# Nielsencu/primal-ppo

Hardware: AMD Instinct MI355X
Metric: agent-steps/sec (env.step+observe) at 4096 envs×8 agents, 1/2/4/8 GPU (higher is better)
Workload: dtype int32; 1 GPU; c2: 4096 envs x 8 agents per GPU, 20x20 warehouse, FOV 11, 6 channels, random policy, env.step+observe; num_envs_per_gpu=4096, num_agents=8, fov=11, channels=6, human=Human (random goals, device A*), goals=lifelong, random, keep_bfs=True, total_envs=4096, parallelism=env-shards x1

## Files before the change

primal-ppo_amd/csrc/mapf_fused_rollout.inc:

```
    extern __shared__ __attribute__((aligned(16))) char smem[];
    constexpr int E = 4;
    constexpr bool TAPE = rollout_pol(POL) == ROLLOUT_TAPE, DESCENT = rollout_pol(POL) == ROLLOUT_DESCENT, PIBT = rollout_pol(POL) == ROLLOUT_PIBT;
    constexpr bool NOISE = rollout_pol_noise(POL);
    const int nb = (int)gridDim.x;
    const int wg = (ro.xcd_remap && (nb & 7) == 0) ? ((int)blockIdx.x & 7) * (nb >> 3) + ((int)blockIdx.x >> 3)
                                                   : (int)blockIdx.x;
    const int sub = SUBS > 1 ? __builtin_amdgcn_readfirstlane((int)(threadIdx.x >> 8)) : 0;
    const int qt = (int)(threadIdx.x & 255);
    const int blk = wg * SUBS + sub;
    const int b0 = blk * E;
    const int nenv = min(E, e.B - b0);
    const int le = qt >> 6;
    char *qsm = smem + (SUBS > 1 ? (size_t)sub * ro.sub_lds : 0);
    uint32_t *prog = reinterpret_cast<uint32_t *>(smem + (size_t)SUBS * ro.sub_lds);
    static_assert(SUBS == 1 || 4 * SUBS == PACE_RING, "the pacing ring takes the place of the per-wave counters");
    const int gw = sub * E + le;
    ObsLds L{};
    if constexpr (PERF) {
        L.rowsz = e.Hp * e.WW;
        L.mapc = reinterpret_cast<uint32_t *>(qsm);
    } else {
        L = obs_layout(e, E, qsm, true);
    }
    const size_t obs_sz = PERF ? rollout_perf_map_lds(e) : rollout_obs_lds(e);
    const size_t base_sz = PERF ? rollout_perf_lds_bytes(e, ROLLOUT_RANDOM) : rollout_lds_bytes(e, ROLLOUT_RANDOM);
    float4 *lut = reinterpret_cast<float4 *>(qsm + rollout_obs_lds(e) - 256);
    if (!PERF && qt < 16) lut[qt] = make_float4((float)(qt & 1), (float)((qt >> 1) & 1), (float)((qt >> 2) & 1), (float)(qt >> 3));
    if (SUBS > 1 && (int)threadIdx.x < 4 * SUBS)
        prog[threadIdx.x] = ro.fair <= 0 || wg * SUBS * E + (int)threadIdx.x < e.B ? 0u : 0xFFFFFFFFu;
    __syncthreads();
    if constexpr (!PERF) L.lut = lut;
    const size_t swl = srch::wave_lds<uint32_t, 1>(e.H, e.W);
    char *slds = qsm + obs_sz + (size_t)le * swl;
    uint32_t *lpath = reinterpret_cast<uint32_t *>(qsm + obs_sz + 4 * swl) + (size_t)le * e.Lmax;
    int32_t *trow = nullptr;
    if constexpr (TAPE) trow = reinterpret_cast<int32_t *>(qsm + base_sz) + (size_t)le * TAPE_K * 8;
    if constexpr (DESCENT || PIBT) trow = reinterpret_cast<int32_t *>(qsm + base_sz) + (size_t)le * 8;
    const uint32_t mreg = obs_map_word(e, b0, nenv, (int)(threadIdx.x & 63));
    EnvRegs rs{};
    if (le < nenv) env_regs_load<8>(e, b0 + le, rs, lpath);
    uint32_t pseen = 0, psince = 0;
    if constexpr (PIBT) {
        if (le < nenv) {
            const size_t ag = (size_t)(b0 + le) * e.N + (size_t)min((int)(threadIdx.x & 63) >> 3, e.N - 1);
            pseen = static_cast<const RO &>(ro).pibt_seen[ag];
            psince = static_cast<const RO &>(ro).pibt_since[ag];
        }
    }
    [[maybe_unused]] PerfAcc pacc;
    if constexpr (PERF) {
        if (le < nenv) pacc = perf_acc_load(ro_perf(ro) + (b0 + __builtin_amdgcn_readfirstlane(le)), ro_accumulate(ro));
    }
    if constexpr (PERF) __builtin_amdgcn_s_waitcnt(0xC07F);
    __builtin_amdgcn_s_waitcnt(0x0F70);
    uint32_t band_mask = 0;
    bool band_moves = false;
    if constexpr (BAND == OBS_BAND) {
        band_moves = ((size_t)e.B * e.N * e.C * e.F * e.F * 4) % MAPF_BAND_UNIT != 0;
        if (le < nenv && !band_moves)
            band_mask = obs_band_skip_mask(e, MAPF_BAND_UNIT, (size_t)(ro.obs + (size_t)(b0 + le) * e.N * e.C * e.F * e.F),
                                           (int)(threadIdx.x & 63));
    }
    if constexpr (PERF) {
        if (le < nenv && (int)(threadIdx.x & 63) < L.rowsz) L.mapc[(size_t)le * L.rowsz + (threadIdx.x & 63)] = mreg;
        __builtin_amdgcn_fence(__ATOMIC_ACQ_REL, "wavefront");
        __builtin_amdgcn_wave_barrier();
    }
    RSTAMP_BEGIN();
    const bool pacing = SUBS > 1 && ro.slack >= 0 && __builtin_amdgcn_readfirstlane(le) < nenv;
    const bool fair = SUBS > 1 && ro.fair > 0 && le < nenv;
    const int live = min(max(e.B - wg * SUBS * E, 0), 4 * SUBS);
    for (int t = 0; t < T; ++t) {
        const DevEnv &E = e;
        const RO &R = ro;
        if (pacing) {
            RSTAMP_WAIT0();
            pace_wait(prog, t, R.slack, live);
            RSTAMP_WAIT1();
        }
        if (fair) {
            if ((uint32_t)t > group_min(prog, 4 * SUBS) + (uint32_t)R.fair) __builtin_amdgcn_s_setprio(0);
            else __builtin_amdgcn_s_setprio(2);
        }
        const size_t BN = (size_t)E.B * E.N;
        const size_t s = R.slots ? (size_t)t : 0;
        [[maybe_unused]] uint32_t *sp_words = nullptr;
        if constexpr (BAND == OBS_SPARSE) {
            const int lew = __builtin_amdgcn_readfirstlane(le);
            sp_words = ro_shadow(ro) + (s * (size_t)E.B + (size_t)(b0 + lew)) * OBS_SPARSE_WORDS;
            band_mask = 0xFFFFFFFFu;
            if (t < ro_valid(ro) && lew < nenv) band_mask = obs_sparse_old(sp_words, (int)(threadIdx.x & 63));
        }
        if constexpr (TAPE) {
            if ((t & (TAPE_K - 1)) == 0) {
                if (le < nenv) {
                    int lane = (int)(threadIdx.x & 63);
                    asm volatile("" : "+v"(lane));
                    const int i = lane & 7, r0 = lane >> 3, nrow = min(TAPE_K, T - t);
                    const int32_t *src = R.actions + ((size_t)(t + r0) * E.B + (size_t)(b0 + le)) * E.N + i;
                    int32_t v[TAPE_K / 8];
#pragma unroll
                    for (int k = 0; k < TAPE_K / 8; ++k)
                        v[k] = (i < E.N && r0 + 8 * k < nrow) ? src[(size_t)(8 * k) * BN] : 0;
#pragma unroll
                    for (int k = 0; k < TAPE_K / 8; ++k) as_lds(trow)[lane + 64 * k] = v[k];
                }
                __builtin_amdgcn_fence(__ATOMIC_ACQ_REL, "wavefront");
                __builtin_amdgcn_wave_barrier();
            }
        }
        if constexpr (DESCENT) {
            __builtin_amdgcn_fence(__ATOMIC_ACQUIRE, "wavefront");
            if (le < nenv) {
                int lane = (int)(threadIdx.x & 63);
                asm volatile("" : "+v"(lane));
                const int i = lane >> 3;
                const bool head = (lane & 7) == 0 && i < E.N;
                int a = 0;
                if (head) {
                    const size_t ai = (size_t)(b0 + le) * E.N + i;
                    a = descent_action(E, E.bfs + ai * bfs_cells(E.H, E.W), rs.pi, rs.clock, i);
                    if (!PERF || R.actions) R.actions[s * BN + ai] = a;
                }
                if constexpr (NOISE)
                    a = noise_play_wave(E.seed, E.env_offset + (uint32_t)(b0 + le), rs.clock, E.noise_q16, E.N, head, i, a);
                if (head) as_lds(trow)[i] = a;
            }
            __builtin_amdgcn_fence(__ATOMIC_ACQ_REL, "wavefront");
            __builtin_amdgcn_wave_barrier();
        }
        if constexpr (PIBT) {
            __builtin_amdgcn_fence(__ATOMIC_ACQUIRE, "wavefront");
            if (le < nenv) {
                int lane = (int)(threadIdx.x & 63);
                asm volatile("" : "+v"(lane));
                const int i = lane >> 3;
                const bool head = (lane & 7) == 0 && i < E.N;
                const size_t ai = (size_t)(b0 + le) * E.N + (size_t)min(i, E.N - 1);
                uint32_t cand[NA] = {PIBT_NONE, PIBT_NONE, PIBT_NONE, PIBT_NONE, PIBT_NONE};
                uint32_t age = 0;
                if (head) {
                    age = pibt_age(pseen, psince, rs.gi, rs.clock);
                    const unsigned sm = E.smask[(E.shared_map ? 0 : (size_t)(b0 + le) * E.H * E.W) + prow(rs.pi) * E.W + pcol(rs.pi)];
                    pibt_candidates(E, E.bfs + ai * bfs_cells(E.H, E.W), rs.pi, sm, rs.hp, rs.hn, rs.clock, i, cand, [&](int j) {
                        return (uint32_t)__builtin_amdgcn_readfirstlane(
                            (int)human_ahead(as_lds(rs.lp), rs.hs, rs.hcur ? rs.hlen1 : rs.hlen0, j));
                    });
                }
                int a = pibt_solve_wave<8>(E.N, lane, head ? rs.pi : NO_CELL, cand, age);
                if (head && (!PERF || R.actions)) R.actions[s * BN + ai] = a;
                if constexpr (NOISE)
                    a = noise_play_wave(E.seed, E.env_offset + (uint32_t)(b0 + le), rs.clock, E.noise_q16, E.N, head, i, a);
                if (head) as_lds(trow)[i] = a;
            }
            __builtin_amdgcn_fence(__ATOMIC_ACQ_REL, "wavefront");
            __builtin_amdgcn_wave_barrier();
        }
        StepOut o = PERF ? StepOut{} : R.out;
        if (o.status) o.status += s * BN;
        if (o.reward) o.reward += s * BN;
        if (o.shadow_goals) o.shadow_goals += s * E.B;
        if (o.cost) o.cost += s * BN;
        if (o.train_valid) o.train_valid += s * BN * NA;
        if (o.actions_fixed) o.actions_fixed += s * BN;
        if (o.goals_reached) o.goals_reached += s * BN;
        if (o.constraints) o.constraints += s * BN;
        if (o.reward_total) o.reward_total += s * BN;
        PairsDeferred dfr;
        [[maybe_unused]] StepVals pv;
        step_pairs_env<8, !PERF, true, true, TAPE || DESCENT || PIBT, PERF>(
            E, TAPE ? trow + (size_t)(t & (TAPE_K - 1)) * 8 : (DESCENT || PIBT ? trow : (PERF && !R.actions ? nullptr : R.actions + s * BN)), o,
            TAPE || DESCENT || PIBT ? 1u : 3u, 0,
            blk * 256 + qt, L, b0, RegMap{mreg, true}, dfr, &rs, PERF ? &pv : nullptr);
        if constexpr (PERF) {
            if (le < nenv) {
                perf_acc_step<8>(pacc, pv, E.N, (int)(threadIdx.x & 63));
                step_pairs_search_inline(E, dfr, slds, L.mapc + (size_t)le * L.rowsz, rs);
            }
        } else
        if (le < nenv) {
            const ObsGroup g = obs_wave_init(E, L, le, mreg);
            if (BAND == OBS_BAND && band_moves)
                band_mask = obs_band_skip_mask(E, MAPF_BAND_UNIT,
                                               (size_t)(R.obs + (s * BN + (size_t)(b0 + le) * E.N) * E.C * E.F * E.F),
                                               (int)(threadIdx.x & 63));
            float *ob;
            if constexpr (ST == OBS_BITS) ob = R.obs + s * BN * (size_t)obs_bits_words(E.C, E.F);
            else ob = R.obs + s * BN * E.C * E.F * E.F;
            obs_emit<false, ST, BAND, PIBT ? 0 : OBS_NT_GROUP>(E, L, ob, R.vec + s * BN * 4, g, b0, false, band_mask);
            if constexpr (BAND == OBS_SPARSE) obs_sparse_store(g.stream, L.swe, sp_words, (int)(threadIdx.x & 63));
            step_pairs_search_inline(E, dfr, slds, L.mapc + (size_t)le * L.rowsz, rs);
            if (pacing) pace_arrive(prog, t);
            else if (fair) publish_count(prog + gw, (uint32_t)(t + 1));
        }
        __builtin_amdgcn_fence(__ATOMIC_ACQ_REL, "wavefront");
        __builtin_amdgcn_wave_barrier();
    }
    if (le < nenv) env_regs_store<8>(e, b0 + le, rs);
    if constexpr (PIBT) {
        const int lane = (int)(threadIdx.x & 63);
        if (le < nenv && (lane & 7) == 0 && (lane >> 3) < e.N) {
            static_cast<const RO &>(ro).pibt_seen[(size_t)(b0 + le) * e.N + (lane >> 3)] = pseen;
            static_cast<const RO &>(ro).pibt_since[(size_t)(b0 + le) * e.N + (lane >> 3)] = psince;
        }
    }
    if constexpr (PERF) {
        if (le < nenv) perf_acc_store(pacc, ro_perf(ro) + (b0 + le), (int)(threadIdx.x & 63));
    }
    if (le < nenv) RSTAMP_END(b0 + le);
```

primal-ppo_amd/csrc/mapf_observe.h:

```cpp
#pragma once
#include "mapf_common.h"
#include "mapf_obs_bits.h"

namespace mapf {

constexpr int OBS_PLAIN = 0, OBS_NT = 1, OBS_BITS = 2;

struct ObsLds {
    int swe;
    uint32_t *stream, *occ, *mapc, *spos, *sgoal, *shn, *shp;
    int32_t *shpn;
    uint8_t *idg;
    uint32_t *bfsw;
    int32_t *bfsown;
    const float4 *lut;
    int stream_words, rowsz;
    bool bfs_win;
};

__host__ __device__ inline int obs_stream_words(const DevEnv &e, int E) { return (E * e.N * e.C * e.F * e.F + 31) / 32 + 1; }

__host__ __device__ inline bool obs_bfs_windows(const DevEnv &e) { return e.C >= 7 && e.keep_bfs && (e.W & 1) == 0; }
__host__ __device__ inline int obs_bfs_wd(const DevEnv &e) { return (e.F + 2) >> 1; }

// ... 122 lines not shown
    if (u0 < o) return false;
    const uint32_t r0 = u0 - o, r1 = r0 + (uint32_t)unit;
    const uint32_t k = r0 / ab;
    return r0 >= k * ab + 4u * (uint32_t)z0 && r1 <= k * ab + 4u * (uint32_t)z1;
}
__host__ __device__ inline int obs_band_iters(const DevEnv &e) { return ((e.N * e.C * e.F * e.F) / 4 + 63) / 64; }
__host__ __device__ inline uint32_t obs_band_skip_mask(const DevEnv &e, int unit, size_t off, int lane) {
    const int nq = (e.N * e.C * e.F * e.F) >> 2;
    uint32_t m = 0;
    for (int k = 0, q = lane; q < nq && k < 32; ++k, q += 64)
        if (obs_band_skip(e, unit, off, q)) m |= 1u << k;
    return m;
}
#ifndef MAPF_BAND_UNIT
#define MAPF_BAND_UNIT 64
#endif

__device__ inline void obs_zero_band_store(const DevEnv &e, float *__restrict__ obs, size_t k0, size_t k1, size_t t,
                                           size_t nt) {
    int z0, z1;
    if (!obs_zero_band(e, z0, z1)) return;
    const size_t CFF = (size_t)e.C * e.F * e.F;
    float4 *o4 = reinterpret_cast<float4 *>(obs);
    const float4 zero = make_float4(0.f, 0.f, 0.f, 0.f);
    for (size_t idx = k0 * 32 + t; idx < k1 * 32; idx += nt) {
        const size_t k = idx >> 5, j = idx & 31;
        const size_t qa = (k * CFF + z0 + 3) >> 2, qb = (k * CFF + z1) >> 2;
        if (qa + j < qb) o4[qa + j] = zero;
    }
}

constexpr int OBS_BAND = 1, OBS_SPARSE = 2;
constexpr int OBS_SPARSE_WORDS = 16, OBS_SPARSE_PIECE = 16;
__host__ __device__ inline bool obs_sparse_applies(int N, int C, int F, size_t obs_addr) {
    const int fl = N * C * F * F;
    return fl > 0 && fl % OBS_SPARSE_PIECE == 0 && fl / OBS_SPARSE_PIECE <= 32 * OBS_SPARSE_WORDS && (obs_addr & 63) == 0;
}
__device__ inline uint32_t obs_sparse_old(const uint32_t *words, int lane) {
    typedef const __attribute__((address_space(4))) uint32_t cu32;
    cu32 *w = (cu32 *)(uintptr_t)words;
    const int g = lane >> 2;
    uint32_t a = 0;
#pragma unroll
    for (int j = 0; j < OBS_SPARSE_WORDS; ++j) a |= ((w[j] >> g) & 0x10001u) << j;
    return a;
}
__device__ inline void obs_sparse_store(const uint32_t *stream, int swe, uint32_t *words, int lane) {
    uint32_t b = 0;
#pragma unroll
    for (int i = 0; i < 4; ++i) {
        const int idx = 4 * lane + i;
        const uint32_t w = idx < swe ? stream[idx] : 0u;
        b |= (((w & 0xFFFFu) ? 1u : 0u) | ((w >> 16) ? 2u : 0u)) << (2 * i);
    }
    b |= (uint32_t)__shfl_down((int)b, 1) << 8;
    b |= (uint32_t)__shfl_down((int)b, 2) << 16;
    if ((lane & 3) == 0) words[lane >> 2] = b;
}

struct ObsGroup {
    int tid, nt;
    int le0, nenv;
    uint32_t *stream;
    const uint32_t *mapc;
    bool wave;
#ifdef MAPF_STAMPS
    int diag = 0;
#endif
};

__device__ inline void obs_sync(const ObsGroup &g) {
    if (g.wave) {
        __builtin_amdgcn_fence(__ATOMIC_ACQ_REL, "wavefront");
        __builtin_amdgcn_wave_barrier();
    } else {
        __syncthreads();
    }
}

__device__ inline ObsGroup obs_workgroup(const ObsLds &L, int nenv) {
    return ObsGroup{(int)threadIdx.x, (int)blockDim.x, 0, nenv, L.stream, L.mapc, false};
}

__device__ inline ObsGroup obs_wave_init(const DevEnv &e, const ObsLds &L, int le, uint32_t mreg) {
    const int lane = lane_id();
    uint32_t *st = L.stream + (size_t)le * L.swe;
    for (int k = lane; k < L.swe; k += 64) st[k] = 0u;
    for (int k = lane; k < L.rowsz; k += 64) L.occ[le * L.rowsz + k] = 0u;
    uint32_t *mp = L.mapc + le * L.rowsz;
    if (lane < L.rowsz) mp[lane] = mreg;
    ObsGroup g{lane, 64, le, 1, st, mp, true};
    obs_sync(g);
    return g;
}

constexpr int OBS_NT_GROUP = 4;
constexpr uint32_t OBS_NT_DROP = 0x80000000u;
constexpr int OBS_NT_AUX = 16 | 2;
#ifndef MAPF_STORE_PRED
#define MAPF_STORE_PRED 0
#endif

template <int BAND, bool WHOLE, int GN>
__device__ __forceinline__ void obs_nt_group(__amdgpu_buffer_rsrc_t rs, const float4 *lut, const uint32_t *swp, int sh,
                                             int hsh, uint32_t voff, uint32_t mask, int cnt) {
    typedef uint32_t v4u __attribute__((ext_vector_type(4)));
    uint32_t sw[GN], vo[GN];
    float4 f[GN];
#pragma unroll
    for (int j = 0; j < GN; ++j) sw[j] = (WHOLE || j < cnt) ? swp[8 * j] : 0u;
#pragma unroll
    for (int j = 0; j < GN; ++j) {
        bool skip = false;
        if constexpr (BAND == OBS_BAND) skip = (mask >> j) & 1u;
        if constexpr (BAND == OBS_SPARSE)
            skip = (__builtin_amdgcn_ubfe(sw[j], hsh, 16) | __builtin_amdgcn_ubfe(mask, (j & 1) * 16 + (j >> 1), 1)) == 0;
        vo[j] = skip ? OBS_NT_DROP : voff;
        if constexpr (BAND != 0) asm("" : "+v"(vo[j]));
    }
#pragma unroll
    for (int j = 0; j < GN; ++j)
        if (WHOLE || j < cnt) f[j] = lut[__builtin_amdgcn_ubfe(sw[j], sh, 4)];
#pragma unroll
    for (int j = 0; j < GN; ++j) {
        if (!(WHOLE || j < cnt)) continue;
        const v4u d = {__float_as_uint(f[j].x), __float_as_uint(f[j].y), __float_as_uint(f[j].z), __float_as_uint(f[j].w)};
#if MAPF_STORE_PRED
        if (vo[j] != OBS_NT_DROP) __builtin_amdgcn_raw_buffer_store_b128(d, rs, voff + 1024u * j, 0, OBS_NT_AUX);
#else
        __builtin_amdgcn_raw_buffer_store_b128(d, rs, vo[j] + 1024u * j, 0, OBS_NT_AUX);
#endif
    }
}

template <int BAND, int GN>
__device__ __forceinline__ void obs_store_wave_nt(const float4 *lut, const uint32_t *swp, int sh, int hsh, float *dst, int q,
                                                  int lane, uint32_t band_mask) {
    const uintptr_t a = reinterpret_cast<uintptr_t>(dst);
    const uint32_t lo = (uint32_t)__builtin_amdgcn_readfirstlane((int)(uint32_t)a);
    const uint32_t hi = (uint32_t)__builtin_amdgcn_readfirstlane((int)(uint32_t)(a >> 32));
    q = __builtin_amdgcn_readfirstlane(q);
    const __amdgpu_buffer_rsrc_t rs =
        __builtin_amdgcn_make_buffer_rsrc(reinterpret_cast<void *>(((uintptr_t)hi << 32) | lo), 0, q * 16, 0x00020000);
    const int iters = (q + 63) >> 6;
    uint32_t voff = (uint32_t)lane * 16u;
    static_assert(GN == OBS_NT_GROUP, "an even group (the sparse mask's layout) within the immediate offset");
    for (int g = 0; g < iters / GN; ++g) {
        obs_nt_group<BAND, true, GN>(rs, lut, swp, sh, hsh, voff, band_mask, GN);
        swp += 8 * GN;
        voff += 1024u * GN;
        band_mask >>= BAND == OBS_SPARSE ? GN / 2 : GN;
    }
    if (iters % GN) obs_nt_group<BAND, false, GN>(rs, lut, swp, sh, hsh, voff, band_mask, iters % GN);
}

template <bool BFSCH = true, int ST = OBS_PLAIN, int BAND = 0, int GN = 0>
__device__ inline void obs_emit(const DevEnv &e, const ObsLds &L, float *__restrict__ obs, float *__restrict__ vec,
                                const ObsGroup &G, int b0, bool skip_band = false, uint32_t band_mask = 0) {
    using namespace obsd;
    const int N = e.N, F = e.F, C = e.C, FF = F * F, CFF = C * FF;
    const int K = G.nenv * N;
    const int kw = G.le0 * N;
    const int rowsz = L.rowsz;
    const int tid = G.tid, nt = G.nt;
    uint32_t *stream = G.stream;
    b0 += G.le0;
    const int E = G.nenv;

    const int HW = e.H * e.W;
#ifdef MAPF_STAMPS
    const int KB = G.diag == 3 ? 0 : K;
#else
    const int KB = K;
#endif
    for (int k = tid; k < KB; k += nt) {
        const int le = G.le0 + k / N;
        const int r = prow(L.spos[kw + k]), c = pcol(L.spos[kw + k]);
        const int rr = r + e.P, cc = c + e.P;
        atomicOr(&L.occ[le * rowsz + rr * e.WW + (cc >> 5)], 1u << (cc & 31));
        L.idg[le * HW + r * e.W + c] = (uint8_t)(k % N);
    }
    const int half = F / 2;
    const size_t bcells = bfs_cells(e.H, e.W);
    if (BFSCH && L.bfs_win) {
        const int WD = obs_bfs_wd(e);
        for (int idx = tid; idx < KB * F * WD; idx += nt) {
            const int task = idx / WD, w = idx - task * WD;
            const int k = task / F, y = task - k * F;
            const int rr = min(max(prow(L.spos[kw + k]) - half + y, 0), e.H - 1);
            const int col = min(max(((pcol(L.spos[kw + k]) - half) & ~1) + 2 * w, 0), e.W - 2);
            const int16_t *bm = e.bfs + ((size_t)b0 * N + k) * bcells;
            L.bfsw[kw * F * WD + idx] = *reinterpret_cast<const uint32_t *>(bm + bfs_at(e.W, rr, col));
        }
        for (int k = tid; k < KB; k += nt)
            L.bfsown[kw + k] = e.bfs[((size_t)b0 * N + k) * bcells + bfs_at(e.W, prow(L.spos[kw + k]), pcol(L.spos[kw + k]))];
    }
    obs_sync(G);

    const int R2 = e.R * e.R;
    for (int task = tid; task < KB * F; task += nt) {
        const int k = task / F, y = task - k * F;
        const int le = G.le0 + k / N;
        const int pr = prow(L.spos[kw + k]), pc = pcol(L.spos[kw + k]);
        const int tr = pr - half, tc = pc - half;
        const int rr = tr + y;
        const int prow_idx = rr + e.P;
        const uint32_t *mrow = G.mapc + (e.shared_map ? 0 : (le - G.le0) * rowsz) + prow_idx * e.WW;
        const uint32_t *orow = L.occ + le * rowsz + prow_idx * e.WW;
        uint32_t seg0 = seg_at(mrow, e.WW, tc + e.P, F);
        uint32_t segA = seg_at(orow, e.WW, tc + e.P, F);
        const uint32_t self = (y == half) ? (1u << half) : 0u;
        const int base = k * CFF + y * F;
        or_bits(stream, base, seg0 | self, F);
        or_bits(stream, base + FF, segA & ~self, F);
        for (uint32_t others = segA & ~self; others; others &= others - 1u) {
            const int cc = tc + __builtin_ctz(others);
            const int kj = le * N + L.idg[le * HW + rr * e.W + cc];
            const int xr = min(max(prow(L.sgoal[kj]), tr), tr + F - 1);
            const int xc = min(max(pcol(L.sgoal[kj]), tc), tc + F - 1);
            set_bit(stream, k * CFF + 3 * FF + (xr - tr) * F + (xc - tc));
        }
        if (e.use_da && rr >= 0 && rr < e.H) {
            const uint32_t hn = L.shn[le];
            const int dy = prow(hn) - rr;
            if (dy * dy <= R2) {
                const int w = isqrt_floor(R2 - dy * dy);
                int c0 = max(max(pcol(hn) - w, 0), tc), c1 = min(min(pcol(hn) + w, e.W - 1), tc + F - 1);
                if (c0 <= c1) {
                    const uint32_t m = ((1u << (c1 - c0 + 1)) - 1u) << (c0 - tc);
                    or_bits(stream, base + 4 * FF, m, F);
                }
            }
        }
        if (BFSCH && L.bfs_win && rr >= 0 && rr < e.H) {
            const int own = L.bfsown[kw + k];
            const uint32_t *win = L.bfsw + ((size_t)kw * F + task) * obs_bfs_wd(e);
            const int c0 = tc & ~1;
            uint32_t m = 0;
            for (int x = 0; x < F; ++x) {
                const int cc = tc + x, wi = cc - c0;
                const int v = (int16_t)(win[wi >> 1] >> ((wi & 1) * 16));
                if (cc >= 0 && cc < e.W && v >= 0 && v < own) m |= 1u << x;
            }
            if (own < 0) m = 0;
            or_bits(stream, base + 6 * FF, m, F);
        } else if (BFSCH && C >= 7 && e.keep_bfs && rr >= 0 && rr < e.H) {
            const size_t ai = (size_t)b0 * N + k;
            const int16_t *bm = e.bfs + ai * bcells;
            const int own = bm[bfs_at(e.W, pr, pc)];
            const int c0 = tc & ~1, cmax = bfs_tw(e.W) * 8 - 2;
            uint32_t wv[9];
#pragma unroll
            for (int w = 0; w < 9; ++w)
                if (2 * w < F + 1)
                    wv[w] = *reinterpret_cast<const uint32_t *>(bm + bfs_at(e.W, rr, min(max(c0 + 2 * w, 0), cmax)));
            uint32_t m = 0;
#pragma unroll
            for (int x = 0; x < 16; ++x) {
                const int cc = tc + x, wi = cc - c0;
                if (x < F) {
                    const int v = (int16_t)(wv[wi >> 1] >> ((wi & 1) * 16));
                    if (cc >= 0 && cc < e.W && v >= 0 && v < own) m |= 1u << x;
                }
            }
            if (own < 0) m = 0;
            or_bits(stream, base + 6 * FF, m, F);
        }
    }

    for (int k = tid; k < KB; k += nt) {
        const int le = G.le0 + k / N;
        const int pr = prow(L.spos[kw + k]), pc = pcol(L.spos[kw + k]);
        const int tr = pr - half, tc = pc - half;
        const int base = k * CFF;
        const int gr = prow(L.sgoal[kw + k]), gc = pcol(L.sgoal[kw + k]);
        if (tr <= gr && gr < tr + F && tc <= gc && gc < tc + F) set_bit(stream, base + 2 * FF + (gr - tr) * F + (gc - tc));
        const uint32_t hn = L.shn[le];
        const int hr = prow(hn), hc = pcol(hn);
        if (tr <= hr && hr < tr + F && tc <= hc && hc < tc + F) set_bit(stream, base + 4 * FF + (hr - tr) * F + (hc - tc));
        for (int q = 0; q < L.shpn[le]; ++q) {
            const uint32_t cell = L.shp[le * e.k_predict + q];
            const int r = prow(cell), c = pcol(cell);
            if (tr <= r && r < tr + F && tc <= c && c < tc + F) set_bit(stream, base + 5 * FF + (r - tr) * F + (c - tc));
        }
        const int dx = gr - pr, dy = gc - pc;
        const int d2 = dx * dx + dy * dy;
        float4 v;
        if (d2 == 0) {
            v = make_float4(0.f, 0.f, 0.f, 0.f);
        } else {
            const double d = __builtin_sqrt((double)d2);
            v = make_float4((float)((double)dx / d), (float)((double)dy / d), (float)d, 0.f);
        }
        reinterpret_cast<float4 *>(vec)[(size_t)b0 * N + k] = v;
    }
    obs_sync(G);
    TL_STAMP(4);
#ifdef MAPF_STAMPS
    if (G.diag == 2) return;
#endif

    if constexpr (ST == OBS_BITS) {
        const int WPA = obs_bits_words(C, F), nw = K * WPA;
        uint32_t *dw = reinterpret_cast<uint32_t *>(obs) + (size_t)b0 * N * WPA;
        if (((N * WPA) & 3) == 0 && ((uintptr_t)dw & 15) == 0) {
            for (int q = tid; q < (nw >> 2); q += nt) {
                int k = (4 * q) / WPA, w = 4 * q - k * WPA;
                uint32_t v[4];
#pragma unroll
                for (int j = 0; j < 4; ++j) {
                    v[j] = obs_bits_word(stream, CFF, k, w);
                    if (++w == WPA) { w = 0; ++k; }
                }
                reinterpret_cast<uint4 *>(dw)[q] = make_uint4(v[0], v[1], v[2], v[3]);
            }
        } else {
            for (int i = tid; i < nw; i += nt) {
                const int k = i / WPA;
                dw[i] = obs_bits_word(stream, CFF, k, i - k * WPA);
            }
        }
        return;
    }
    const size_t total = (size_t)K * CFF;
    float *dst = obs + (size_t)b0 * N * CFF;
    if (G.wave && L.lut && !skip_band && ((K * CFF) & 3) == 0) {
        const int sh = (tid & 7) * 4;
        const uint32_t *swp = stream + (tid >> 3);
        if constexpr (ST == OBS_NT && GN != 0) {
            obs_store_wave_nt<BAND, GN>(L.lut, swp, sh, (tid & 4) * 4, dst, (K * CFF) >> 2, tid, band_mask);
            return;
        }
        float4 *dp = reinterpret_cast<float4 *>(dst) + tid;
        [[maybe_unused]] int it = 0;
#pragma unroll 4
        for (int rem = ((K * CFF) >> 2) - tid; rem > 0; rem -= 64) {
            const uint32_t sw = *swp;
            const float4 f = L.lut[__builtin_amdgcn_ubfe(sw, sh, 4)];
            bool skip = false;
            if constexpr (BAND == OBS_BAND) skip = band_mask & 1u;
            if constexpr (BAND == OBS_SPARSE)
                skip = (__builtin_amdgcn_ubfe(sw, (tid & 4) * 4, 16) | __builtin_amdgcn_ubfe(band_mask, (it & 1) * 16 + (it >> 1), 1)) == 0;
            if (skip) {
            } else if constexpr (ST == OBS_NT) {
                typedef float v4f __attribute__((ext_vector_type(4)));
#if defined(MAPF_SLOT_STORE) && MAPF_SLOT_STORE == 1
                __builtin_nontemporal_store(v4f{f.x, f.y, f.z, f.w}, reinterpret_cast<v4f *>(dp));
#elif defined(MAPF_SLOT_STORE) && MAPF_SLOT_STORE == 2
                asm volatile("global_store_dwordx4 %0, %1, off sc1\n\ts_nop 1" ::"v"(dp), "v"(v4f{f.x, f.y, f.z, f.w}) : "memory");
#elif defined(MAPF_SLOT_STORE) && MAPF_SLOT_STORE == 3
                *dp = f;
#else
// ... 65 lines not shown
```

primal-ppo_amd/csrc/mapf_step_pairs.h:

```cpp
#pragma once
#include "mapf_group.h"
#include "mapf_kernels.h"
#include "mapf_observe.h"
#include "mapf_pyset.h"

namespace mapf {

namespace pairs {

__device__ inline unsigned abit(int r, int c) {
    if (r == 0 && c == 0) return 1u;
    if (r == 0 && c == 1) return 1u << 1;
    if (r == 1 && c == 0) return 1u << 2;
    if (r == 0 && c == -1) return 1u << 3;
    if (r == -1 && c == 0) return 1u << 4;
    return 0u;
}
__device__ inline unsigned keys_of(int r, int c) {
    unsigned m = 0;
#pragma unroll
    for (int t = 0; t < NA; ++t)
        if (abs(dr(t) - r) + abs(dc(t) - c) <= 1) m |= 1u << t;
    return m;
}
// ... 19 lines not shown
struct EnvRegs {
    uint32_t pi, pj, gi;
    int la;
    float creg;
    uint32_t clock, hp, hn, hng, hgoal, hstart, hentr, replans;
    int hs, hcur, hlen0, hlen1;
    uint32_t *lp;
};

__device__ inline void env_regs_path_to_lds(const DevEnv &e, int b, int buf, int len, uint32_t *lp) {
    const uint32_t *p = human_path(e, b, buf);
    for (int k = lane_id(); k < len; k += 64) lp[k] = p[k];
    __builtin_amdgcn_fence(__ATOMIC_ACQ_REL, "wavefront");
    __builtin_amdgcn_wave_barrier();
}

template <int NP>
__device__ inline void env_regs_load(const DevEnv &e, int b, EnvRegs &r, uint32_t *lp) {
    const int lane = lane_id(), i = lane / NP, j = lane % NP;
    const bool vi = i < e.N, vj = j < e.N;
    const size_t ai = (size_t)b * e.N + i, aj = (size_t)b * e.N + j;
    r.pi = vi ? e.pos[ai] : 0u;
    r.pj = vj ? e.pos[aj] : 0u;
    r.gi = vi ? e.goal[ai] : 0u;
    r.la = vi ? (int)e.last_act[ai] : -1;
    const int RR = e.R * e.R;
    r.creg = RR < 64 ? e.cost_lut[lane <= RR ? lane : 0] : 0.f;
    r.clock = e.clock[b];
    r.hentr = e.hentr[b];
    r.hp = e.hpos[b];
    r.hn = e.hnext[b];
    r.hng = e.hnext_goal[b];
    r.hgoal = e.hgoal[b];
    r.hstart = e.hnext_start[b];
    r.replans = 0u;
    r.hs = e.hstep[b];
    r.hcur = e.hcur[b];
    r.hlen0 = e.hlen[(size_t)b * 2];
    r.hlen1 = e.hlen[(size_t)b * 2 + 1];
    r.lp = lp;
    env_regs_path_to_lds(e, b, r.hcur, r.hcur ? r.hlen1 : r.hlen0, lp);
}

template <int NP>
__device__ inline void env_regs_store(const DevEnv &e, int b, const EnvRegs &r) {
    const int lane = lane_id(), i = lane / NP, j = lane % NP;
    if (i < e.N && j == 0) {
        const size_t ai = (size_t)b * e.N + i;
        e.pos[ai] = r.pi;
        e.goal[ai] = r.gi;
        e.last_act[ai] = (int8_t)r.la;
    }
    if (lane == 0) {
        e.clock[b] = r.clock;
        e.hpos[b] = r.hp;
        e.hnext[b] = r.hn;
        e.hnext_goal[b] = r.hng;
        e.hgoal[b] = r.hgoal;
        e.hnext_start[b] = r.hstart;
        e.hreplans[b] += r.replans;
        e.hstep[b] = r.hs;
        e.hcur[b] = r.hcur;
    }
}

__device__ inline void step_pairs_finish(const DevEnv &e, const PairsDeferred &d, int slot) {
    const int lane = lane_id();
    if (d.bmask) {
        const uint32_t base = __builtin_amdgcn_readlane(d.bret, __builtin_ctzll(d.bmask));
        if ((d.bmask >> lane) & 1ull)
            e.bfs_list[(size_t)slot * e.B * e.N + base + __popcll(d.bmask & ((1ull << lane) - 1ull))] = d.bitem;
    }
    if (d.rmask) {
        const uint32_t base = __builtin_amdgcn_readlane(d.rret, __builtin_ctzll(d.rmask));
        if ((d.rmask >> lane) & 1ull)
            e.replan_list[(size_t)slot * e.B + base + __popcll(d.rmask & ((1ull << lane) - 1ull))] = d.ritem;
    }
}

template <int NP, bool FEED, bool INLINE = false, bool RES = false, bool LDSACT = false, bool PERF = false>
__device__ __forceinline__ void step_pairs_env(const DevEnv &e, int32_t *__restrict__ actions, const StepOut &out,
                                               uint32_t flags, int slot, int gt, const ObsLds &ob, int b0,
                                               RegMap rm, PairsDeferred &dfr, EnvRegs *rs = nullptr,
                                               StepVals *pv = nullptr) {
    using namespace pairs;
    constexpr int L = NP * NP;
    constexpr uint32_t ROW = (1u << NP) - 1u;
    const int N = e.N;
    const int b = (L == 64) ? __builtin_amdgcn_readfirstlane(gt / L) : gt / L;
    if (!INLINE && gt == 0 && (flags & 1u)) {
        e.counters[C_REPLAN_COUNT + (slot + 1) % 3] = 0;
        e.counters[C_BFS_COUNT + (slot + 1) % 3] = 0;
    }
    if (b >= e.B) return;
    STAMP_BEGIN();
    const int lane = lane_id();
    const int base = lane & ~(L - 1), li = lane - base;
    const int i = li / NP, j = li % NP;
    const uint64_t emask = (L == 64) ? ~0ull : (((1ull << L) - 1ull) << base);
    auto eballot = [&](bool p) -> uint64_t { return (__ballot(p) & emask) >> base; };
    auto agents_of = [&](uint64_t m) -> uint32_t {
        if constexpr (NP == 8) {
            m &= 0x0101010101010101ull;
            m |= m >> 7;
            m |= m >> 14;
            m |= m >> 28;
            return (uint32_t)m & 0xFFu;
        }
        uint32_t a = 0;
#pragma unroll
        for (int k = 0; k < NP; ++k) a |= (uint32_t)((m >> (k * NP)) & 1ull) << k;
        return a;
    };
    const bool vi = i < N, vj = j < N;
    const bool head = j == 0;
    const size_t ai = (size_t)b * N + i, aj = (size_t)b * N + j;
    const uint32_t env_id = e.env_offset + (uint32_t)b;
    const uint32_t clock = RES ? rs->clock : e.clock[b];
    const int RR = e.R * e.R;
    const bool lutreg = L == 64 && RR < 64;
    const float creg = !lutreg ? 0.f : RES ? rs->creg : e.cost_lut[lane_id() <= RR ? lane_id() : 0];
    const uint32_t hp = RES ? rs->hp : e.hpos[b], hn = RES ? rs->hn : e.hnext[b];
    const int hs = RES ? rs->hs : e.hstep[b], hcur = RES ? rs->hcur : e.hcur[b];
    const int2 hlen2 = RES ? make_int2(rs->hlen0, rs->hlen1) : *reinterpret_cast<const int2 *>(e.hlen + (size_t)b * 2);
    const int hmode = RES ? (e.human_mode == 1 ? 1 : 0) : e.human_mode;
    const int gmode = RES ? 1 : e.goal_mode;
    const uint32_t hng = hmode == 1 ? (RES ? rs->hng : e.hnext_goal[b]) : NO_CELL;
    const int hsi = hmode == 2 ? e.hseq_idx[b] : 0, hsl = hmode == 2 ? e.hseq_len[b] : 0;

    const uint32_t pi = RES ? rs->pi : (vi ? e.pos[ai] : 0u), pj = RES ? rs->pj : (vj ? e.pos[aj] : 0u);
    const int ri = prow(pi), ci = pcol(pi), rj = prow(pj), cj = pcol(pj);
    const uint32_t gi = RES ? rs->gi : (vi ? e.goal[ai] : 0u);
    const int la = RES ? rs->la : (vi ? (int)e.last_act[ai] : -1);
    int a_i, a_j;
    if (flags & 2u) {
        const u32x4 o = philox(env_id, P_ACT, clock, 0u, e.seed);
        a_i = random_action(o, i);
        a_j = random_action(o, j);
        if (vi && head && (!PERF || actions)) actions[ai] = a_i;
    } else {
        if constexpr (LDSACT) {
            const auto row = as_lds(actions);
            a_i = vi ? row[i] : 0;
            a_j = vj ? row[j] : 0;
        } else {
            a_i = vi ? actions[ai] : 0;
            a_j = vj ? actions[aj] : 0;
        }
        if (vi && head && (a_i < 0 || a_i >= NA)) atomicAdd(&e.counters[C_BAD_ACTION], 1u);
        if (a_i < 0 || a_i >= NA) a_i = 0;
        if (a_j < 0 || a_j >= NA) a_j = 0;
    }
    const int Lc = hcur ? hlen2.y : hlen2.x;
    int cur2 = hcur, hs2 = hs + 1, seq_idx = 0;
    bool swapped = false, at_end = hs >= Lc - 1;
    if (at_end) {
        hs2 = 0;
        if (hmode == 1) {
            if (hng != NO_CELL) { cur2 = hcur ^ 1; swapped = true; }
        } else if (hmode == 2) {
            seq_idx = hsi + 1;
            if (seq_idx < hsl) { cur2 = hcur ^ 1; swapped = true; }
        }
    }
    const int L2 = cur2 ? hlen2.y : hlen2.x;
    const uint32_t *p2 = human_path(e, b, cur2);
    if (RES && cur2 != hcur) env_regs_path_to_lds(e, b, cur2, L2, rs->lp);
    const uint32_t *p2r = RES ? rs->lp : p2;
    const uint32_t hp_new = p2r[hs2];
    const uint32_t hn_new = p2r[hs2 + 1 < L2 ? hs2 + 1 : L2 - 1];
    unsigned st_mask = 0x1Fu;
    if (rm.on) {
        unsigned m = 0;
#pragma unroll
        for (int k = 1; k < NA; ++k) m |= (unsigned)rm.obstacle(e, nullptr, ri + dr(k), ci + dc(k)) << k;
        if (vi) st_mask = m;
    } else if (vi) {
        st_mask = (unsigned)e.smask[(e.shared_map ? 0 : (size_t)b * e.H * e.W) + ri * e.W + ci];
    }
    unsigned hu_mask = 0;
#pragma unroll
    for (int k = 0; k < NA; ++k) {
        if ((st_mask >> k) & 1u) continue;
        const uint32_t x = pack(ri + dr(k), ci + dc(k));
        if (x == hn || (pi == hn && x == hp)) hu_mask |= 1u << k;
    }
    const unsigned rep_mask = la >= 0 ? 1u << opp(la) : 0u;
    STAMP(0);

    unsigned kij = 0, cij = 0;
    if (vi && vj && i != j) {
        const int r = rj - ri, c = cj - ci;
        if (abs(r) + abs(c) <= 2) {
            kij = keys_of(r, c);
            const int er = r + dr(a_j), ec = c + dc(a_j);
            cij = abit(er, ec);
            if (er == 0 && ec == 0) cij |= abit(r, c);
        }
    }
    const uint64_t Mb = eballot((cij >> a_i) & 1u);
    const uint32_t kc = row_or<NP>(kij | (cij << 8));
    const unsigned keys = kc & 0x1Fu, conf = (kc >> 8) & 0x1Fu;
    const unsigned good = ~(st_mask | hu_mask | rep_mask | keys) & 0x1Fu;
    const uint32_t Mi = (uint32_t)(Mb >> (i * NP)) & ROW;
    STAMP(1);

    int s0;
    bool cb = false;
    if ((st_mask >> a_i) & 1u) s0 = -1;
    else if ((hu_mask >> a_i) & 1u) s0 = -2;
    else if ((good >> a_i) & 1u) s0 = 1;
    else if (Mi) { s0 = -3; cb = true; }
    else s0 = ((rep_mask >> a_i) & 1u) ? -4 : 1;
    const uint32_t cbm = agents_of(eballot(head && vi && cb));
    uint32_t T = 0;
    for (uint32_t rem = cbm; rem; rem &= rem - 1) {
        const int k = __builtin_ctz(rem);
        if (!((T >> k) & 1u)) T |= ((uint32_t)(Mb >> (k * NP)) & ROW) | (1u << k);
    }
    const int st = ((T >> i) & 1u) ? -3 : s0;

    float c_act = e.action_cost, c_rep = e.repeat_cost, c_col = e.collision_cost, c_hum = e.human_collision_cost;
    asm volatile("" : "+s"(c_act), "+s"(c_rep), "+s"(c_col), "+s"(c_hum));
    float rw = c_act;
    rw = st == -4 ? c_rep : rw;
    rw = (st == -1 || st == -3) ? c_col : rw;
    rw = st == -2 ? c_hum : rw;
    const int Xr = ri + dr(a_i), Xc = ci + dc(a_i);
    const uint32_t shadow = agents_of(eballot(head && vi && st == 1 && Xr == prow(gi) && Xc == pcol(gi)));
    float cost = 0.f;
    {
        const int d0 = prow(hn) - Xr, d1 = pcol(hn) - Xc;
        const int d2 = d0 * d0 + d1 * d1;
        if (lutreg) {
            const float c = __shfl(creg, d2 < RR ? d2 : 0, 64);
            cost = d2 < RR ? c : 0.f;
        } else if (d2 < RR) {
            cost = (float)(((double)e.R - sqrt((double)d2)) / (double)e.R);
        }
    }
    if (vi) {
        if (head) {
            if (out.status) out.status[ai] = (int8_t)st;
            if (out.reward) out.reward[ai] = rw;
            if (out.cost) out.cost[ai] = cost;
        }
        if (out.train_valid) {
            float *tv = out.train_valid + ai * NA;
            for (int t = j; t < NA; t += NP)
                tv[t] = (((good >> t) & 1u) || (((keys >> t) & 1u) && !((conf >> t) & 1u))) ? 1.f : 0.f;
        }
    }
    if (li == 0 && out.shadow_goals) out.shadow_goals[b] = __popc(shadow);
    if constexpr (PERF) {
        if (vi && head) { pv->st = st; pv->cost = cost; }
        pv->nshadow = __popc(shadow);
    }
    STAMP(2);
    if (!(flags & 1u)) return;

    int fixed = a_i;
    const uint32_t need = agents_of(eballot(head && vi && (st == -1 || st == -2 || st == -3)));
    if (need) {
        const int st_j = (int)shfl32((uint32_t)st, base + j * NP);
        const unsigned good_j = shfl32(good, base + j * NP);
        int asg_i = (vi && st == 1) ? a_i : -1;
        int asg_j = (vj && st_j == 1) ? a_j : -1;
        if (vi && st < 0 && good) asg_i = __builtin_ctz(good);
        if (vj && st_j < 0 && good_j) asg_j = __builtin_ctz(good_j);
        const uint32_t qm = agents_of(eballot(head && vi && st < 0 && !good));
        int q = (vi && st < 0 && !good) ? __popc(qm & ((1u << i) - 1u)) : -1;
        int next_q = __popc(qm), hd = 0, draws = 0;
        const unsigned viable_i = ~(st_mask | hu_mask) & 0x1Fu;
        while (hd < next_q) {
            const int idx = __builtin_ctz(agents_of(eballot(head && vi && q == hd)));
            const unsigned good_idx = shfl32(good, base + idx * NP);
            int newa = -1;
            uint32_t ev = 0;
            bool swap_ev = false;
            if (good_idx) {
                newa = __builtin_ctz(good_idx);
            } else {
                const unsigned viable = shfl32(viable_i, base + idx * NP);
                unsigned cjm = 0;
                if (i == idx && vj && j != idx && asg_j >= 0) {
                    const int r = rj - ri, c = cj - ci;
                    if (abs(r) + abs(c) <= 2) {
                        const int er = r + dr(asg_j), ec = c + dc(asg_j);
                        cjm = abit(er, ec);
                        if (er == 0 && ec == 0) cjm |= abit(r, c);
                    }
                }
                unsigned U = 0;
#pragma unroll
                for (int t = 0; t < NA; ++t)
                    if (eballot((cjm >> t) & 1u)) U |= 1u << t;
                const unsigned fr = viable & ~U;
                if (fr) {
                    newa = __builtin_ctz(fr);
                } else {
                    if (draws >= fix_draws(N)) {
                        if (li == 0) atomicAdd(&e.counters[C_FIX_BOUND], 1u);
                        break;
                    }
                    const int nv = __popc(viable);
                    newa = 0;
                    if (nv == 0) {
                        if (li == 0) atomicAdd(&e.counters[C_EMPTY_VIABLE], 1u);
                    } else {
                        int pick;
                        if (e.fix_choice == 0) pick = draws % nv;
                        else pick = (int)__umulhi(philox(env_id, P_FIX | ((uint32_t)idx << 8), clock, (uint32_t)draws,
                                                         e.seed).x, (uint32_t)nv);
                        newa = nth_bit(viable, pick);
                    }
                    ++draws;
                    ev = (uint32_t)(eballot((cjm >> newa) & 1u) >> (idx * NP)) & ROW;
                    if (__builtin_expect(__popc(ev) == 2, 0)) {
                        unsigned rb = 0;
                        if (i == idx && vj && j != idx) {
                            const int Xr = ri + dr(newa), Xc = ci + dc(newa);
#pragma unroll
                            for (int t = 0; t < NA; ++t) {
                                const int yr = rj + dr(t), yc = cj + dc(t);
                                if ((yr == Xr && yc == Xc) || (Xr == rj && Xc == cj && yr == ri && yc == ci)) rb |= 1u << t;
                            }
                        }
                        const unsigned rbk = shfl32(rb, base + idx * NP + (li < NP ? li : 0));
                        const int ja = __builtin_ctz(ev), jb = 31 - __builtin_clz(ev);
                        const int asg_k = li < NP ? asg_j : -1;
                        if constexpr (L == 64) {
                            const int ba = __builtin_amdgcn_readlane(asg_j, ja), bb = __builtin_amdgcn_readlane(asg_j, jb);
                            swap_ev = evict_pair_swapped(WaveGroup(), N, li < NP ? rbk : 0u, asg_k, ja, ba, jb, bb);
                        } else {
                            const int ba = (int)shfl32((uint32_t)asg_j, base + ja), bb = (int)shfl32((uint32_t)asg_j, base + jb);
                            swap_ev = evict_pair_swapped(Group(L), N, li < NP ? rbk : 0u, asg_k, ja, ba, jb, bb);
// ... 60 lines not shown
            if (!group_free_cell(e, env_id, P_GOAL, k, clock, ok, r, c)) {
                if (li == 0) atomicAdd(&e.counters[C_FREECELL], 1u);
                const uint32_t npk = shfl32(np, base + k * NP);
                r = prow(npk); c = pcol(npk);
            }
            if (i == k) ng = pack(r, c);
        }
    }
    if constexpr (RES) {
        if (vi) { rs->pi = np; rs->gi = ng; rs->la = fixed; }
        const uint32_t npj = shfl32(np, base + j * NP);
        if (vj) rs->pj = npj;
    } else if (vi && head) {
        e.pos[ai] = np;
        e.goal[ai] = ng;
        e.last_act[ai] = (int8_t)fixed;
    }
    if (e.keep_bfs) {
        const uint64_t bm = __ballot(vi && head && reached);
        if (bm) {
            if (!INLINE && lane == __builtin_ctzll(bm))
                dfr.bret = atomicAdd(&e.counters[C_BFS_COUNT + slot], (uint32_t)__popcll(bm));
            dfr.bmask = bm;
            dfr.bitem = (uint32_t)ai;
            dfr.bgoal = ng;
        }
    }
    STAMP(4);

    if (at_end) {
        if (hmode == 1) {
            if (RES) {
                if (swapped) { rs->hgoal = hng; rs->replans += 1u; }
            } else if (swapped && li == 0) {
                e.hgoal[b] = hng; e.hreplans[b] += 1u;
            }
        } else if (hmode == 2) {
            if (li == 0) {
                e.hgoal[b] = e.hseq[(size_t)b * e.HS + (seq_idx < hsl ? seq_idx : hsl - 1)];
                e.hseq_idx[b] = seq_idx;
            }
        }
    }
    if (swapped) {
        uint32_t ns, ngl;
        plan_next_path(e, b, env_id, clock + (uint32_t)L2, seq_idx, ns, ngl, li == 0, rm, hmode,
                       RES ? rs->hentr : 0u, RES);
        if (RES) {
            rs->hstart = ns;
            rs->hng = ngl;
        } else if (li == 0) {
            e.hnext_start[b] = ns;
            e.hnext_goal[b] = ngl;
        }
        const uint64_t rmk = __ballot(li == 0 && ngl != NO_CELL);
        if (rmk) {
            if (!INLINE && lane == __builtin_ctzll(rmk))
                dfr.rret = atomicAdd(&e.counters[C_REPLAN_COUNT + slot], (uint32_t)__popcll(rmk));
            dfr.rmask = rmk;
            dfr.ritem = (uint32_t)b;
            dfr.rstart = ns;
            dfr.rgoal = ngl;
            dfr.rbuf = cur2 ^ 1;
        }
    }
    if (RES) {
        rs->hcur = cur2;
        rs->hs = hs2;
        rs->hp = hp_new;
        rs->hn = hn_new;
        rs->clock = clock + 1u;
    } else if (li == 0) {
        e.hcur[b] = cur2;
        e.hstep[b] = hs2;
        e.hpos[b] = hp_new;
        e.hnext[b] = hn_new;
        e.clock[b] = clock + 1u;
    }
    STAMP(5);

    if (vi && head) {
        const int d0 = prow(hp_new) - nr, d1 = pcol(hp_new) - nc;
        const float cv = (d0 * d0 + d1 * d1 <= e.constr_d2) ? 1.f : 0.f;
        if (out.actions_fixed) out.actions_fixed[ai] = fixed;
        if (out.goals_reached) out.goals_reached[ai] = reached ? 1.f : 0.f;
        if (out.constraints) out.constraints[ai] = cv;
        if (out.reward_total) out.reward_total[ai] = reached ? rw + e.goal_reward : rw;
        if constexpr (PERF) {
            pv->reached = reached;
            pv->cv = cv == 1.f;
            pv->rtot = reached ? rw + e.goal_reward : rw;
        }
    }
    STAMP(6);
    if constexpr (FEED) {
        const int le = b - b0;
        if (vi && head) {
            ob.spos[le * N + i] = np;
            ob.sgoal[le * N + i] = ng;
        }
        if (li == 0) ob.shn[le] = hn_new;
        if (e.use_hp && e.C >= 6) {
            const int kp = e.k_predict;
            for (int q = 1 + li; q <= kp && q < L2; q += L) ob.shp[le * kp + q - 1] = p2r[q];
            if (li == 0) ob.shpn[le] = min(kp, L2 - 1);
        } else if (li == 0) {
            ob.shpn[le] = 0;
        }
    }
    STAMP_END();
}

}
```

Before: 2.605 billion agent-steps/s.

## Add lean one-wave observation path with hoisted map copy and fused offsets

```diff
diff --git a/primal-ppo_amd/csrc/mapf_fused_rollout.inc b/primal-ppo_amd/csrc/mapf_fused_rollout.inc
--- a/primal-ppo_amd/csrc/mapf_fused_rollout.inc
+++ b/primal-ppo_amd/csrc/mapf_fused_rollout.inc
@@ -1,6 +1,7 @@
     extern __shared__ __attribute__((aligned(16))) char smem[];
     constexpr int E = 4;
     constexpr bool TAPE = rollout_pol(POL) == ROLLOUT_TAPE, DESCENT = rollout_pol(POL) == ROLLOUT_DESCENT, PIBT = rollout_pol(POL) == ROLLOUT_PIBT;
+    constexpr bool LEAN = !PIBT && ST != OBS_PLAIN;
     constexpr bool NOISE = rollout_pol_noise(POL);
     const int nb = (int)gridDim.x;
     const int wg = (ro.xcd_remap && (nb & 7) == 0) ? ((int)blockIdx.x & 7) * (nb >> 3) + ((int)blockIdx.x >> 3)
@@ -61,8 +62,8 @@
             band_mask = obs_band_skip_mask(e, MAPF_BAND_UNIT, (size_t)(ro.obs + (size_t)(b0 + le) * e.N * e.C * e.F * e.F),
                                            (int)(threadIdx.x & 63));
     }
-    if constexpr (PERF) {
-        if (le < nenv && (int)(threadIdx.x & 63) < L.rowsz) L.mapc[(size_t)le * L.rowsz + (threadIdx.x & 63)] = mreg;
+    if constexpr (PERF || LEAN) {
+        if (le < nenv) obs_wave_map(L, le, mreg);
         __builtin_amdgcn_fence(__ATOMIC_ACQ_REL, "wavefront");
         __builtin_amdgcn_wave_barrier();
     }
@@ -157,21 +158,23 @@
             __builtin_amdgcn_wave_barrier();
         }
         StepOut o = PERF ? StepOut{} : R.out;
-        if (o.status) o.status += s * BN;
-        if (o.reward) o.reward += s * BN;
-        if (o.shadow_goals) o.shadow_goals += s * E.B;
-        if (o.cost) o.cost += s * BN;
-        if (o.train_valid) o.train_valid += s * BN * NA;
-        if (o.actions_fixed) o.actions_fixed += s * BN;
-        if (o.goals_reached) o.goals_reached += s * BN;
-        if (o.constraints) o.constraints += s * BN;
-        if (o.reward_total) o.reward_total += s * BN;
+        if constexpr (!LEAN) {
+            if (o.status) o.status += s * BN;
+            if (o.reward) o.reward += s * BN;
+            if (o.shadow_goals) o.shadow_goals += s * E.B;
+            if (o.cost) o.cost += s * BN;
+            if (o.train_valid) o.train_valid += s * BN * NA;
+            if (o.actions_fixed) o.actions_fixed += s * BN;
+            if (o.goals_reached) o.goals_reached += s * BN;
+            if (o.constraints) o.constraints += s * BN;
+            if (o.reward_total) o.reward_total += s * BN;
+        }
         PairsDeferred dfr;
         [[maybe_unused]] StepVals pv;
         step_pairs_env<8, !PERF, true, true, TAPE || DESCENT || PIBT, PERF>(
             E, TAPE ? trow + (size_t)(t & (TAPE_K - 1)) * 8 : (DESCENT || PIBT ? trow : (PERF && !R.actions ? nullptr : R.actions + s * BN)), o,
             TAPE || DESCENT || PIBT ? 1u : 3u, 0,
-            blk * 256 + qt, L, b0, RegMap{mreg, true}, dfr, &rs, PERF ? &pv : nullptr);
+            blk * 256 + qt, L, b0, RegMap{mreg, true}, dfr, &rs, PERF ? &pv : nullptr, LEAN ? s * BN : 0, LEAN ? s * (size_t)E.B : 0);
         if constexpr (PERF) {
             if (le < nenv) {
                 perf_acc_step<8>(pacc, pv, E.N, (int)(threadIdx.x & 63));
@@ -179,7 +182,7 @@
             }
         } else
         if (le < nenv) {
-            const ObsGroup g = obs_wave_init(E, L, le, mreg);
+            const ObsGroup g = obs_wave_init(E, L, le, mreg, !LEAN, LEAN);
             if (BAND == OBS_BAND && band_moves)
                 band_mask = obs_band_skip_mask(E, MAPF_BAND_UNIT,
                                                (size_t)(R.obs + (s * BN + (size_t)(b0 + le) * E.N) * E.C * E.F * E.F),
@@ -187,7 +190,7 @@
             float *ob;
             if constexpr (ST == OBS_BITS) ob = R.obs + s * BN * (size_t)obs_bits_words(E.C, E.F);
             else ob = R.obs + s * BN * E.C * E.F * E.F;
-            obs_emit<false, ST, BAND, PIBT ? 0 : OBS_NT_GROUP>(E, L, ob, R.vec + s * BN * 4, g, b0, false, band_mask);
+            obs_emit<false, ST, BAND, PIBT ? 0 : OBS_NT_GROUP, LEAN>(E, L, ob, R.vec + s * BN * 4, g, b0, false, band_mask);
             if constexpr (BAND == OBS_SPARSE) obs_sparse_store(g.stream, L.swe, sp_words, (int)(threadIdx.x & 63));
             step_pairs_search_inline(E, dfr, slds, L.mapc + (size_t)le * L.rowsz, rs);
             if (pacing) pace_arrive(prog, t);
diff --git a/primal-ppo_amd/csrc/mapf_observe.h b/primal-ppo_amd/csrc/mapf_observe.h
--- a/primal-ppo_amd/csrc/mapf_observe.h
+++ b/primal-ppo_amd/csrc/mapf_observe.h
@@ -228,13 +228,23 @@
     return ObsGroup{(int)threadIdx.x, (int)blockDim.x, 0, nenv, L.stream, L.mapc, false};
 }
 
-__device__ inline ObsGroup obs_wave_init(const DevEnv &e, const ObsLds &L, int le, uint32_t mreg) {
+__device__ inline void obs_wave_map(const ObsLds &L, int le, uint32_t mreg) {
+    const int lane = lane_id();
+    if (lane < L.rowsz) L.mapc[le * L.rowsz + lane] = mreg;
+}
+__device__ inline ObsGroup obs_wave_init(const DevEnv &e, const ObsLds &L, int le, uint32_t mreg, bool copy_map = true,
+                                         bool zero16 = false) {
     const int lane = lane_id();
     uint32_t *st = L.stream + (size_t)le * L.swe;
-    for (int k = lane; k < L.swe; k += 64) st[k] = 0u;
+    if (zero16) {
+        uint4 *st4 = reinterpret_cast<uint4 *>(st);
+        for (int k = lane; k < (L.swe >> 2); k += 64) st4[k] = make_uint4(0u, 0u, 0u, 0u);
+    } else {
+        for (int k = lane; k < L.swe; k += 64) st[k] = 0u;
+    }
     for (int k = lane; k < L.rowsz; k += 64) L.occ[le * L.rowsz + k] = 0u;
     uint32_t *mp = L.mapc + le * L.rowsz;
-    if (lane < L.rowsz) mp[lane] = mreg;
+    if (copy_map) obs_wave_map(L, le, mreg);
     ObsGroup g{lane, 64, le, 1, st, mp, true};
     obs_sync(g);
     return g;
@@ -300,7 +310,85 @@
     if (iters % GN) obs_nt_group<BAND, false, GN>(rs, lut, swp, sh, hsh, voff, band_mask, iters % GN);
 }
 
-template <bool BFSCH = true, int ST = OBS_PLAIN, int BAND = 0, int GN = 0>
+__device__ inline void obs_wave_occ(const DevEnv &e, const ObsLds &L, const ObsGroup &G, int KB) {
+    const int k = G.tid >> 3;
+    if ((G.tid & 7) == 0 && k < KB) {
+        const uint32_t p = L.spos[G.le0 * e.N + k];
+        const int r = prow(p), c = pcol(p);
+        const int rr = r + e.P, cc = c + e.P;
+        atomicOr(&L.occ[G.le0 * L.rowsz + rr * e.WW + (cc >> 5)], 1u << (cc & 31));
+        L.idg[G.le0 * e.H * e.W + r * e.W + c] = (uint8_t)k;
+    }
+}
+
+__device__ inline void obs_wave_rows(const DevEnv &e, const ObsLds &L, float *__restrict__ vec, const ObsGroup &G,
+                                     int b, int KB) {
+    using namespace obsd;
+    const int k = G.tid >> 3, j = G.tid & 7;
+    if (k >= KB) return;
+    const int N = e.N, F = e.F, FF = F * F, half = F / 2;
+    const int le = G.le0, kw = le * N;
+    uint32_t *stream = G.stream;
+    const uint32_t *occ = L.occ + le * L.rowsz;
+    const uint8_t *idg = L.idg + le * e.H * e.W;
+    const uint32_t p = L.spos[kw + k];
+    const int pr = prow(p), pc = pcol(p);
+    const int tr = pr - half, tc = pc - half;
+    const int abase = k * (e.C * FF);
+    const int R2 = e.R * e.R;
+    for (int y0 = 0; y0 < F; y0 += 8) {
+        const int y = y0 + j;
+        if (y >= F) continue;
+        const int rr = tr + y;
+        const int prow_idx = rr + e.P;
+        const uint32_t seg0 = seg_at(G.mapc + prow_idx * e.WW, e.WW, tc + e.P, F);
+        const uint32_t segA = seg_at(occ + prow_idx * e.WW, e.WW, tc + e.P, F);
+        const uint32_t self = (y == half) ? (1u << half) : 0u;
+        const int base = abase + y * F;
+        or_bits(stream, base, seg0 | self, F);
+        or_bits(stream, base + FF, segA & ~self, F);
+        for (uint32_t others = segA & ~self; others; others &= others - 1u) {
+            const int cc = tc + __builtin_ctz(others);
+            const uint32_t g = L.sgoal[kw + idg[rr * e.W + cc]];
+            const int xr = min(max(prow(g), tr), tr + F - 1);
+            const int xc = min(max(pcol(g), tc), tc + F - 1);
+            set_bit(stream, abase + 3 * FF + (xr - tr) * F + (xc - tc));
+        }
+        if (e.use_da && rr >= 0 && rr < e.H) {
+            const uint32_t hn = L.shn[le];
+            const int dy = prow(hn) - rr;
+            if (dy * dy <= R2) {
+                const int w = isqrt_floor(R2 - dy * dy);
+                const int c0 = max(max(pcol(hn) - w, 0), tc), c1 = min(min(pcol(hn) + w, e.W - 1), tc + F - 1);
+                if (c0 <= c1) or_bits(stream, base + 4 * FF, ((1u << (c1 - c0 + 1)) - 1u) << (c0 - tc), F);
+            }
+        }
+    }
+    if (j != 0) return;
+    const uint32_t gl = L.sgoal[kw + k];
+    const int gr = prow(gl), gc = pcol(gl);
+    if (tr <= gr && gr < tr + F && tc <= gc && gc < tc + F) set_bit(stream, abase + 2 * FF + (gr - tr) * F + (gc - tc));
+    const uint32_t hn = L.shn[le];
+    const int hr = prow(hn), hc = pcol(hn);
+    if (tr <= hr && hr < tr + F && tc <= hc && hc < tc + F) set_bit(stream, abase + 4 * FF + (hr - tr) * F + (hc - tc));
+    for (int q = 0; q < L.shpn[le]; ++q) {
+        const uint32_t cell = L.shp[le * e.k_predict + q];
+        const int r = prow(cell), c = pcol(cell);
+        if (tr <= r && r < tr + F && tc <= c && c < tc + F) set_bit(stream, abase + 5 * FF + (r - tr) * F + (c - tc));
+    }
+    const int dx = gr - pr, dy = gc - pc;
+    const int d2 = dx * dx + dy * dy;
+    float4 v;
+    if (d2 == 0) {
+        v = make_float4(0.f, 0.f, 0.f, 0.f);
+    } else {
+        const double d = __builtin_sqrt((double)d2);
+        v = make_float4((float)((double)dx / d), (float)((double)dy / d), (float)d, 0.f);
+    }
+    reinterpret_cast<float4 *>(vec)[(size_t)b * N + k] = v;
+}
+
+template <bool BFSCH = true, int ST = OBS_PLAIN, int BAND = 0, int GN = 0, bool WV = false>
 __device__ inline void obs_emit(const DevEnv &e, const ObsLds &L, float *__restrict__ obs, float *__restrict__ vec,
                                 const ObsGroup &G, int b0, bool skip_band = false, uint32_t band_mask = 0) {
     using namespace obsd;
@@ -319,6 +407,9 @@
 #else
     const int KB = K;
 #endif
+    static_assert(!(WV && BFSCH), "the one-wave path has no BFS channel");
+    if constexpr (WV) obs_wave_occ(e, L, G, KB);
+    else
     for (int k = tid; k < KB; k += nt) {
         const int le = G.le0 + k / N;
         const int r = prow(L.spos[kw + k]), c = pcol(L.spos[kw + k]);
@@ -344,6 +435,8 @@
     obs_sync(G);
 
     const int R2 = e.R * e.R;
+    if constexpr (WV) obs_wave_rows(e, L, vec, G, b0, KB);
+    else
     for (int task = tid; task < KB * F; task += nt) {
         const int k = task / F, y = task - k * F;
         const int le = G.le0 + k / N;
@@ -414,6 +507,7 @@
         }
     }
 
+    if constexpr (!WV)
     for (int k = tid; k < KB; k += nt) {
         const int le = G.le0 + k / N;
         const int pr = prow(L.spos[kw + k]), pc = pcol(L.spos[kw + k]);
diff --git a/primal-ppo_amd/csrc/mapf_step_pairs.h b/primal-ppo_amd/csrc/mapf_step_pairs.h
--- a/primal-ppo_amd/csrc/mapf_step_pairs.h
+++ b/primal-ppo_amd/csrc/mapf_step_pairs.h
@@ -125,7 +125,7 @@
 __device__ __forceinline__ void step_pairs_env(const DevEnv &e, int32_t *__restrict__ actions, const StepOut &out,
                                                uint32_t flags, int slot, int gt, const ObsLds &ob, int b0,
                                                RegMap rm, PairsDeferred &dfr, EnvRegs *rs = nullptr,
-                                               StepVals *pv = nullptr) {
+                                               StepVals *pv = nullptr, size_t so = 0, size_t sb = 0) {
     using namespace pairs;
     constexpr int L = NP * NP;
     constexpr uint32_t ROW = (1u << NP) - 1u;
@@ -158,6 +158,7 @@
     const bool vi = i < N, vj = j < N;
     const bool head = j == 0;
     const size_t ai = (size_t)b * N + i, aj = (size_t)b * N + j;
+    const size_t ao = ai + so;
     const uint32_t env_id = e.env_offset + (uint32_t)b;
     const uint32_t clock = RES ? rs->clock : e.clock[b];
     const int RR = e.R * e.R;
@@ -284,17 +285,17 @@
     }
     if (vi) {
         if (head) {
-            if (out.status) out.status[ai] = (int8_t)st;
-            if (out.reward) out.reward[ai] = rw;
-            if (out.cost) out.cost[ai] = cost;
+            if (out.status) out.status[ao] = (int8_t)st;
+            if (out.reward) out.reward[ao] = rw;
+            if (out.cost) out.cost[ao] = cost;
         }
         if (out.train_valid) {
-            float *tv = out.train_valid + ai * NA;
+            float *tv = out.train_valid + ao * NA;
             for (int t = j; t < NA; t += NP)
                 tv[t] = (((good >> t) & 1u) || (((keys >> t) & 1u) && !((conf >> t) & 1u))) ? 1.f : 0.f;
         }
     }
-    if (li == 0 && out.shadow_goals) out.shadow_goals[b] = __popc(shadow);
+    if (li == 0 && out.shadow_goals) out.shadow_goals[(size_t)b + sb] = __popc(shadow);
     if constexpr (PERF) {
         if (vi && head) { pv->st = st; pv->cost = cost; }
         pv->nshadow = __popc(shadow);
@@ -521,10 +522,10 @@
     if (vi && head) {
         const int d0 = prow(hp_new) - nr, d1 = pcol(hp_new) - nc;
         const float cv = (d0 * d0 + d1 * d1 <= e.constr_d2) ? 1.f : 0.f;
-        if (out.actions_fixed) out.actions_fixed[ai] = fixed;
-        if (out.goals_reached) out.goals_reached[ai] = reached ? 1.f : 0.f;
-        if (out.constraints) out.constraints[ai] = cv;
-        if (out.reward_total) out.reward_total[ai] = reached ? rw + e.goal_reward : rw;
+        if (out.actions_fixed) out.actions_fixed[ao] = fixed;
+        if (out.goals_reached) out.goals_reached[ao] = reached ? 1.f : 0.f;
+        if (out.constraints) out.constraints[ao] = cv;
+        if (out.reward_total) out.reward_total[ao] = reached ? rw + e.goal_reward : rw;
         if constexpr (PERF) {
             pv->reached = reached;
             pv->cv = cv == 1.f;
```

Result: faster. 2.855 billion agent-steps/s (median of 6 runs) (+9.6%).
